# ericzzj1989/BALF

Measured on NVIDIA B200. Metric: images/sec detect+NMS+top-k @640x480, higher is better.
Workload: dtype fp16/tf32 operands (11-bit significand), fp32 accumulate

## Files before the change

### balf_b200/csrc/detector.cu

```cuda
#include <cuda_fp16.h>
#include "detector.cuh"

namespace balf {

constexpr int NT = 256;
constexpr int kWbufFloats = 4096;

enum { ACT_NONE = 0, ACT_RELU = 1, ACT_GELU = 2, ACT_LRELU = 3 };

template <int ACT> __device__ __forceinline__ float act_fn(float v) {
    if (ACT == ACT_RELU) return fmaxf(v, 0.0f);
    if (ACT == ACT_GELU) return 0.5f * v * (1.0f + erff(v * 0.70710678118654752440f));
    if (ACT == ACT_LRELU) return v > 0.0f ? v : 0.2f * v;
    return v;
}


template <int M, int K, int N, int ACT, bool ALIAS>
__device__ __forceinline__ void linear_tile(const float* in_s, const float* __restrict__ wT, int ldw,
                                            const float* __restrict__ bias, float* out_s, const float* res_s,
                                            float* wbuf) {
    constexpr int MP = M + 4;
    constexpr int TMB = M / 8, NTH = NT / TMB;
    constexpr int NC = N < NTH * 8 ? N : NTH * 8;
// ... 303 lines not shown
        float o = __ldg(w.ex2_b + c);
        for (int k = 0; k < C / 4; ++k) o = fmaf(hid[k], __ldg(w.ex2_w + (size_t)k * C + c), o);
        scale[(size_t)b * C + c] = 1.0f / (1.0f + expf(-o));
    }
}

template <int C, int swz, bool OH>
__global__ void pool_kernel(const float* __restrict__ r, const float* __restrict__ q, const float* __restrict__ scale,
                            int h, int w, float* __restrict__ out, size_t total) {
    size_t i = (size_t)blockIdx.x * blockDim.x + threadIdx.x;
    if (i >= total) return;
    constexpr int Q = C / 4;
    const int c4 = (int)(i % Q);
    size_t t = i / Q;
    const int wo = w / 2, ho = h / 2;
    const int px = (int)(t % wo);
    t /= wo;
    const int py = (int)(t % ho);
    const size_t b = t / ho;
    const float4 s = __ldg(reinterpret_cast<const float4*>(scale + b * C) + c4);
    float4 best = make_float4(kNegInf, kNegInf, kNegInf, kNegInf);
#pragma unroll
    for (int dy = 0; dy < 2; ++dy)
#pragma unroll
        for (int dx = 0; dx < 2; ++dx) {
            size_t p = (b * h + 2 * py + dy) * w + 2 * px + dx;
            const size_t rowi = p & 127;
            const size_t cs = (swz == 1 || swz == 2) ? (((p - rowi) * C) >> 2) + (size_t)(c4 >> 3) * (128 * 8) + rowi * 8 + ((c4 & 7) ^ (rowi & 7))
                                  : ((p * C) >> 2) + c4;
            float4 rv;
            if constexpr (swz == 1) {
                const uint2 h = __ldg(reinterpret_cast<const uint2*>(reinterpret_cast<const __half*>(r) + (p - rowi) * C +
                                                                     (size_t)(c4 >> 1) * (128 * 8) + rowi * 8 + (c4 & 1) * 4));
                const float2 lo = __half22float2(*reinterpret_cast<const __half2*>(&h.x)), hi = __half22float2(*reinterpret_cast<const __half2*>(&h.y));
                rv = make_float4(lo.x, lo.y, hi.x, hi.y);
            } else if constexpr (swz == 3) {
                const uint2 h = __ldg(reinterpret_cast<const uint2*>(reinterpret_cast<const __half*>(r) + p * C) + c4);
                const float2 lo = __half22float2(*reinterpret_cast<const __half2*>(&h.x)), hi = __half22float2(*reinterpret_cast<const __half2*>(&h.y));
                rv = make_float4(lo.x, lo.y, hi.x, hi.y);
            } else {
                rv = __ldg(reinterpret_cast<const float4*>(r) + cs);
            }
            float4 qv;
            if constexpr (swz == 1) {
                const unsigned char* qt = reinterpret_cast<const unsigned char*>(q) + (p - rowi) * C * 3;
                const uint2 t16 = __ldg(reinterpret_cast<const uint2*>(qt + ((size_t)(c4 >> 1) * 128 + rowi) * 16 + (c4 & 1) * 8));
                const uint32_t m8 = __ldg(reinterpret_cast<const uint32_t*>(qt + (size_t)128 * C * 2 + ((size_t)(c4 >> 2) * 128 + rowi) * 16 + (c4 & 3) * 4));
                qv.x = __uint_as_float(((t16.x & 0xFFFFu) << 16) | ((m8 & 0xFFu) << 8));
                qv.y = __uint_as_float((t16.x & 0xFFFF0000u) | (m8 & 0xFF00u));
                qv.z = __uint_as_float(((t16.y & 0xFFFFu) << 16) | ((m8 >> 8) & 0xFF00u));
                qv.w = __uint_as_float((t16.y & 0xFFFF0000u) | ((m8 >> 16) & 0xFF00u));
            } else {
                qv = __ldg(reinterpret_cast<const float4*>(q) + cs);
            }
            best.x = fmaxf(best.x, rv.x * s.x + qv.x); best.y = fmaxf(best.y, rv.y * s.y + qv.y);
            best.z = fmaxf(best.z, rv.z * s.z + qv.z); best.w = fmaxf(best.w, rv.w * s.w + qv.w);
        }
    if constexpr (OH) {
        uint2 o;
// ... 195 lines not shown
    {
        ProfScope p("det_se", st);
        se_kernel<C><<<Bc, kSeThreads, 0, st>>>(ws.partial, parts, 1.0f / (float)npix, w, ws.scale);
    }
    BALF_COUNT_LAUNCH(1);
    BALF_LAUNCH_OK();
    return 0;
}

template <int C>
static int run_pool(const Workspace& ws, int Bc, int h, int wd, float* out, cudaStream_t st, int swz = 0, bool oh = false) {
    size_t total = (size_t)Bc * (h / 2) * (wd / 2) * (C / 4);
    {
        ProfScope p("det_pool", st);
        const unsigned grid = (unsigned)((total + 255) / 256);
        if (swz == 1 && oh) pool_kernel<C, 1, true><<<grid, 256, 0, st>>>(ws.r, ws.q, ws.scale, h, wd, out, total);
        else if (swz == 1) pool_kernel<C, 1, false><<<grid, 256, 0, st>>>(ws.r, ws.q, ws.scale, h, wd, out, total);
        else if (swz == 2) pool_kernel<C, 2, false><<<grid, 256, 0, st>>>(ws.r, ws.q, ws.scale, h, wd, out, total);
        else if (swz == 3 && oh) pool_kernel<C, 3, true><<<grid, 256, 0, st>>>(ws.r, ws.q, ws.scale, h, wd, out, total);
        else if (swz == 3) pool_kernel<C, 3, false><<<grid, 256, 0, st>>>(ws.r, ws.q, ws.scale, h, wd, out, total);
        else if (oh) pool_kernel<C, 0, true><<<grid, 256, 0, st>>>(ws.r, ws.q, ws.scale, h, wd, out, total);
        else pool_kernel<C, 0, false><<<grid, 256, 0, st>>>(ws.r, ws.q, ws.scale, h, wd, out, total);
    }
    BALF_COUNT_LAUNCH(1);
    BALF_LAUNCH_OK();
    return 0;
}

}

using namespace balf;
// ... 96 lines not shown
    Workspace ws;
    ws_layout(a, chunk, Hp, Wp, workspace, &ws);
    const int nl = a.cell * a.cell + 1, hc = Hp / 8, wc = Wp / 8;
    if (int e = set_smem(head_kernel<256, 32>, HeadSmem<256, 32>::bytes)) return e;
    for (int b0 = 0; b0 < B; b0 += chunk) {
        const int Bc = B - b0 < chunk ? B - b0 : chunk;
        const float* xb = x + (size_t)b0 * 3 * Hp * Wp;
        const int tcm = precision >= 1 ? g_tc_mask : 0;
        const int px = precision == 2 ? 1 : 0;
        const DownW* d = w.down;
        int tiles = 0;
        if (tcm & 1) {
            if (int e = tc_run_level_dispatch(0, xb, true, d[0], a, tc_blob, Bc, Hp, Wp, ws.u, ws.v, ws.r, ws.q, ws.partial, st, px, 0)) return e;
            if (int e = run_se<32>(ws, d[0], Bc, Hp * Wp, Hp * Wp / 64, st)) return e;
        } else if (int e = run_level<3, 32, 128, 128>(xb, true, w.down[0], Bc, Hp, Wp, ws, st, &tiles)) return e;
        if (int e = run_pool<32>(ws, Bc, Hp, Wp, ws.pooled[0], st, (tcm & 1) ? 1 + px : 0, (tcm & 2) && !px)) return e;
        if (tcm & 2) {
            if (int e = tc_run_level_dispatch(1, ws.pooled[0], false, d[1], a, tc_blob, Bc, Hp / 2, Wp / 2, ws.u, ws.v, ws.r, ws.q, ws.partial, st, px, 0)) return e;
            if (int e = run_se<64>(ws, d[1], Bc, Hp * Wp / 4, Hp * Wp / 256, st)) return e;
        } else if (int e = run_level<32, 64, 128, 128>(ws.pooled[0], false, w.down[1], Bc, Hp / 2, Wp / 2, ws, st, &tiles)) return e;
        if (int e = run_pool<64>(ws, Bc, Hp / 2, Wp / 2, ws.pooled[1], st, (tcm & 2) ? 1 + px : 0, (tcm & 4) && !px)) return e;
        if (tcm & 4) {
            if (int e = tc_run_level_dispatch(2, ws.pooled[1], false, d[2], a, tc_blob, Bc, Hp / 4, Wp / 4, ws.u, ws.v, ws.r, ws.q, ws.partial, st, px, px == 0)) return e;
            if (int e = run_se<128>(ws, d[2], Bc, Hp * Wp / 16, Hp * Wp / 1024, st)) return e;
        } else if (int e = run_level<64, 128, 64, 64>(ws.pooled[1], false, w.down[2], Bc, Hp / 4, Wp / 4, ws, st, &tiles)) return e;
        if (int e = run_pool<128>(ws, Bc, Hp / 4, Wp / 4, ws.pooled[2], st, ((tcm & 4) && !px) ? 3 : 0, (tcm & 8) && !px)) return e;
        if (tcm & 8) {
            if (int e = tc_run_level_dispatch(3, ws.pooled[2], false, d[3], a, tc_blob, Bc, hc, wc, ws.u, ws.v, ws.r, ws.q, ws.partial, st, px, px == 0 && (tcm & 16) != 0)) return e;
            if (int e = run_se<256>(ws, d[3], Bc, hc * wc, hc * wc / 64, st)) return e;
        } else if (int e = run_level<128, 256, 64, 32>(ws.pooled[2], false, w.down[3], Bc, hc, wc, ws, st, &tiles)) return e;
        if (tcm & 16) {
// ... 17 lines not shown
```

### balf_b200/csrc/detector.cuh

```cuda
#pragma once
#include "common.cuh"
#include "../../include/balf_b200.h"

namespace balf {

constexpr int kHeadPad = 128;

struct DownW {
    const float *conv0_w, *conv0_b;
    const float *pn_w, *pn_b;
    const float *pd1_w, *pd1_b;
    struct Branch {
        const float *n_w, *n_b;
        const float *d1_w, *d1_b;
        const float *gn_w, *gn_b;
        const float *gd_w, *gd_b;
        const float *d2_w, *d2_b;
    } br[2];
    const float *pd2_w, *pd2_b;
    const float *rn_w, *rn_b;
    const float *rc1_w, *rc1_b, *rc2_w, *rc2_b;
    const float *ex0_w, *ex0_b;
    const float *ex2_w, *ex2_b;
    const float *c2_w, *c2_b;
// ... 37 lines not shown
        d.pd2_w = c.take(2 * ch * ch); d.pd2_b = c.take(ch);
        d.rn_w = c.take(ch); d.rn_b = c.take(ch);
        d.rc1_w = c.take(ch * ch); d.rc1_b = c.take(ch);
        d.rc2_w = c.take(ch * ch); d.rc2_b = c.take(ch);
        d.ex0_w = c.take(ch * red); d.ex0_b = c.take(red);
        d.ex2_w = c.take(red * ch); d.ex2_b = c.take(ch);
        d.c2_w = c.take(ch * ch); d.c2_b = c.take(ch);
    }
    const size_t cl = a.dims[4];
    w.head.w = c.take(cl * kHeadPad); w.head.b = c.take(kHeadPad);
    w.head.alpha = c.take(kHeadPad); w.head.beta = c.take(kHeadPad);
    if (out) *out = w;
    return c.off;
}

size_t tc_blob_floats(const balf_detector_arch& a);
int tc_pack_weights(const balf_detector_arch& a, const DetW& w, float* blob, cudaStream_t st);
int tc_run_level_dispatch(int level, const float* xin, bool nchw, const DownW& w, const balf_detector_arch& a, const float* blob,
                          int Bc, int h, int wd, float* u, float* v, float* r, float* q, float* partial, cudaStream_t st, int px, int r16);
int tc_run_head(const float* r, const float* q, const float* scale, const DownW& w, const HeadW& hw, const balf_detector_arch& a,
                const float* blob, int Bc, int hc, int wc, float* logits, float* prob, cudaStream_t st, int px, int r16);

}
```

### balf_b200/csrc/detector_tc.cuh

```cuda
#pragma once
#include <cuda_fp16.h>
#include "detector.cuh"
#include "umma.cuh"

namespace balf {
using namespace umma;

#ifndef BALF_EXP
#define BALF_EXP 0
#endif
#ifndef BALF_MERGE32_CTAS
#define BALF_MERGE32_CTAS 3
#endif
#ifndef BALF_MERGE_TPR
#define BALF_MERGE_TPR 2
#endif
#ifndef BALF_RC16_MINC
#define BALF_RC16_MINC 32
#endif
constexpr int TM = 128;
constexpr int NT2 = 256;
constexpr int kMaxSlot = 4;
constexpr int kMaxGemm = 6;

struct TcGemm {
    uint32_t goff;
    uint16_t nblk;
    uint16_t rows;
    uint16_t kb;
    uint16_t bias;
    uint16_t h16;
};
__host__ __device__ constexpr uint32_t tc_eb(int h16) { return h16 == 1 ? 2u : 4u; }
struct TcPlan {
    const float* base;
    TcGemm g[kMaxGemm];
    int ngemm;
    int resident;
// ... 108 lines not shown
};
template <int CIN, int C, int PX = 0> struct MergeG {
    static constexpr int count = MG_COUNT;
    static constexpr bool x3 = PX != 0;
    static constexpr bool ebias = C == 128 && PX == 0;
    static constexpr bool resident = PX ? C <= 32 : C <= 128;
    static constexpr int cap = 32768;
    static constexpr int nslot = PX ? (C == 64 ? 3 : 2) : (C == 256 ? 2 : 3);
    __host__ __device__ static constexpr int rows(int) { return C; }
    __host__ __device__ static constexpr int K(int gi) { return gi == MG_CONV0 ? tc_kin(CIN) : C; }
    __host__ __device__ static constexpr bool bias(int gi) { return !ebias && gi != MG_PD2A; }
    __host__ __device__ static constexpr bool h16(int gi) {
        return gi == MG_PD2A || gi == MG_PD2B || (gi == MG_CONV0 && CIN >= 8) || ((gi == MG_RC1 || gi == MG_RC2) && (PX || C > BALF_RC16_MINC));
    }
};
template <int C, int PX = 0> struct HeadG {
    static constexpr int count = HG_COUNT;
    static constexpr bool x3 = PX != 0;
    static constexpr bool resident = false;
    static constexpr int cap = 32768;
    static constexpr int nslot = 2;
    __host__ __device__ static constexpr int rows(int gi) { return gi == HG_DENSE ? kHeadN : C; }
    __host__ __device__ static constexpr int K(int) { return C; }
    __host__ __device__ static constexpr bool bias(int) { return true; }
    __host__ __device__ static constexpr bool h16(int) { return true; }
};
template <typename G> __host__ __device__ constexpr int g_mode(int gi) { return G::h16(gi) ? (G::x3 ? 2 : 1) : 0; }
template <typename G> __host__ __device__ constexpr uint32_t g_bytes(int gi) {
    return (uint32_t)G::rows(gi) * (G::K(gi) * tc_eb(g_mode<G>(gi)) + (G::bias(gi) ? 32u : 0u));
}
// ... 824 lines not shown
                const float mix_b1 = *mix_b1p;
                const unsigned long long b2 = pk2(mix_b1, mix_b1);
#pragma unroll
                for (int i = 0; i < SC; i += 2) upk2(mul2(pk2(y1[i], y1[i + 1]), add2(pk2(y2[i], y2[i + 1]), b2)), y2[i], y2[i + 1]);
                row_to_a16<SC, LOC>(y2, s.region, row, col0 + c);
            }
        }
        TC_TRACE(plan, it, 13);
        sync_for_mma<NG, NTG>(grp);
        if (!(BALF_EXP & 16) && w0 && elect_one()) { issue_linear_t<G, BG_D2>(ring, plan, region_addr, ones_addr, tm + Cfg::col_y, true); commit(s.done); }
        TC_TRACE(plan, it, 14);
        wait_done_ring<G, NG, NTG, Cfg::WW>(s.done, phase, ring, plan, w0, grp);
        TC_TRACE(plan, it, 15);
        {
            const bool odd = (threadIdx.x & 1) != 0;
            const size_t own_base = (Cfg::swz_out || Cfg::h16_out) ? ((size_t)img * npix + (pix & ~(TM - 1))) * C * (Cfg::h16_out && X3 ? 2 : 1)
                                                                   : ((size_t)img * npix + pix) * C;
            const int own_sw = pix & (TM - 1);
            const size_t oth_base = __shfl_xor_sync(0xffffffffu, (unsigned long long)own_base, 1);
            const int oth_sw = __shfl_xor_sync(0xffffffffu, own_sw, 1);
            const size_t base_a = odd ? oth_base : own_base, base_b = odd ? own_base : oth_base;
            const int sw_a = odd ? oth_sw : own_sw, sw_b = odd ? own_sw : oth_sw;
            if constexpr (CL16 && CH % 64 == 0) {
                float hv[CH / 2];
#pragma unroll
                for (int c = 0; c < CH; c += SC) {
                    float a[SC];
                    ld_row<SC>(lane_base + Cfg::col_y + col0 + c, a);
#pragma unroll
                    for (int j0 = 0; j0 < SC / 4; j0 += 8) {
                        float4 t8[8];
                        pair_load<8>(reinterpret_cast<const float4*>(orow + c) + j0, valid, t8);
#pragma unroll
// ... 366 lines not shown
    tc_finish(tm, Cfg::ncols);
}


template <int CIN, int C, int PX = 0> struct MergeBulkCfg {
    static constexpr int CH = C / 2;
    static constexpr bool cc0 = CIN < 8;
    static constexpr uint32_t tile_bytes = (uint32_t)TM * C * 4;
    static constexpr uint32_t uv_bytes = (uint32_t)TM * C * (PX ? 4u : 2u);
    static constexpr uint32_t r16_bytes = 0u;
    static constexpr uint32_t xbytes = cc0 ? 0u : (uint32_t)TM * tc_kin(CIN) * 4;
    static constexpr uint32_t region = 2 * uv_bytes + r16_bytes + 2 * tile_bytes + xbytes;
    static constexpr uint32_t xch = 2u * TM * 8u;
    static constexpr int col_acc = 0, col_x0 = C;
    static constexpr int ncols = tc_cols(cc0 ? C : 2 * C);
    static constexpr int min_ctas = C <= 32 ? (PX ? 2 : BALF_MERGE32_CTAS) : 1;
};

template <int CIN, int C, int PX = 0>
__global__ void __launch_bounds__(NT2, MergeBulkCfg<CIN, C, PX>::min_ctas)
tc_merge_bulk_kernel(const float* __restrict__ xin, DownW w, TcPlan plan, UnitGeom geo, const float* __restrict__ uin,
                     const float* __restrict__ vin, float* __restrict__ rout, float* __restrict__ qout, float* __restrict__ partial) {
    extern __shared__ __align__(1024) unsigned char smem[];
    using Cfg = MergeBulkCfg<CIN, C, PX>;
    constexpr int CH = Cfg::CH;
    using G = MergeG<CIN, C, PX>;
    constexpr int HM = PX ? 2 : 1, LOC = PX ? C / 8 : 0;
    constexpr bool XH = PX == 0 && CIN >= 8;
    constexpr int XM = XH ? 3 : HM;
    const TcShared s = carve(smem, Cfg::region, plan, 1, Cfg::xch);
    float* const regU = s.region;
// ... 165 lines not shown
            }
#pragma unroll
            for (int o = TPP / 2; o >= 1; o >>= 1) {
                acc.x += __shfl_xor_sync(0xffffffffu, acc.x, o);
                acc.y += __shfl_xor_sync(0xffffffffu, acc.y, o);
                acc.z += __shfl_xor_sync(0xffffffffu, acc.z, o);
                acc.w += __shfl_xor_sync(0xffffffffu, acc.w, o);
            }
            if (sub == 0) *reinterpret_cast<float4*>(partial + (size_t)(2 * t + uu) * C + ch * 4) = acc;
        }
    }
    if (w0 && elect_one()) bulk_wait_all();
    tc_finish(tm, Cfg::ncols);
}

template <int C, int PX = 0>
__global__ void __launch_bounds__(NT2, 1) tc_head_kernel(const float* __restrict__ r, const float* __restrict__ q,
                                                         const float* __restrict__ scale, TcPlan plan, UnitGeom geo, int cell,
                                                         float* __restrict__ logits, float* __restrict__ prob, int r16) {
    extern __shared__ __align__(1024) unsigned char smem[];
    using G = HeadG<C, PX>;
    constexpr int LOC = PX ? C / 8 : 0;
    constexpr uint32_t region_bytes = (uint32_t)TM * C * 4;
    constexpr int ncols = tc_cols(C + 96);
    constexpr int CH = C / 2;
    const TcShared s = carve(smem, region_bytes, plan);
    const int tid = threadIdx.x, row = tid & (TM - 1), half = tid >> 7;
    const int ntiles = (geo.total_units + 1) / 2;
    const uint32_t my_tiles = blockIdx.x < (unsigned)ntiles ? (ntiles - 1 - blockIdx.x) / gridDim.x + 1 : 0;
    Ring ring;
// ... 362 lines not shown
}


#ifdef BALF_TC_MAIN
int g_tc_variant = 0x41;
#else
extern int g_tc_variant;
#endif

template <int CIN, int C, int V, int PX>
static int tc_launch_branches(const float* xin, const DownW& w, const TcPlans& P, int level, const UnitGeom& g, int ntiles,
                              float* u, float* v, float* su, float* sv, cudaStream_t st) {
    using Cfg = typename BranchSel<C, V, PX>::Cfg;
    constexpr int NG = Cfg::groups;
    int grid = 0;
    for (int b = 0; b < 2; ++b) {
        const TcPlan& p = P.branch[level][b];
        const size_t smem = tc_smem_bytes(Cfg::region, p, NG, Cfg::xch);
        if (b == 0) {
            if (int e = tc_launch_cfg(tc_branch_kernel<CIN, C, 0, V, PX>, smem, tc_cols(Cfg::ncols * NG), ntiles, &grid, NG, Cfg::NTG)) return e;
            ProfScope ps(C == 32 ? "det_branch_grid_c32" : C == 64 ? "det_branch_grid_c64" : C == 128 ? "det_branch_grid_c128" : "det_branch_grid_c256", st);
            tc_branch_kernel<CIN, C, 0, V, PX><<<grid, Cfg::NTG * NG, smem, st>>>(xin, w, p, g, u, su);
        } else {
            if (int e = tc_launch_cfg(tc_branch_kernel<CIN, C, 1, V, PX>, smem, tc_cols(Cfg::ncols * NG), ntiles, &grid, NG, Cfg::NTG)) return e;
            ProfScope ps(C == 32 ? "det_branch_block_c32" : C == 64 ? "det_branch_block_c64" : C == 128 ? "det_branch_block_c128" : "det_branch_block_c256", st);
            tc_branch_kernel<CIN, C, 1, V, PX><<<grid, Cfg::NTG * NG, smem, st>>>(xin, w, p, g, v, sv);
        }
    }
    return 0;
}
template <int CIN, int C, int PX>
static int tc_run_branches(const float* xin, const DownW& w, const TcPlans& P, int level, const UnitGeom& g, int ntiles,
                           float* u, float* v, float* su, float* sv, cudaStream_t st) {
    const int var = (g_tc_variant >> (2 * level)) & 3;
    if constexpr (C == 32) {
        if (var == 1) return tc_launch_branches<CIN, C, 1, PX>(xin, w, P, level, g, ntiles, u, v, su, sv, st);
        if (var == 2) return tc_launch_branches<CIN, C, 2, PX>(xin, w, P, level, g, ntiles, u, v, su, sv, st);
    }
    if constexpr (C == 64 || C == 128 || C == 256) {
        if (var == 1) return tc_launch_branches<CIN, C, 1, PX>(xin, w, P, level, g, ntiles, u, v, su, sv, st);
    }
    return tc_launch_branches<CIN, C, 0, PX>(xin, w, P, level, g, ntiles, u, v, su, sv, st);
}

template <int CIN, int C, int PX>
static int tc_run_level(const float* xin, const DownW& w, const TcPlans& P, int level, int Bc, int h, int wd,
                        float* u, float* v, float* r, float* q, float* partial, cudaStream_t st, int r16) {
    (void)r16;
    UnitGeom g{h, wd, h / 8, wd / 8, h * wd / 64, Bc * (h * wd / 64), 1.0f / (float)(h * wd / 64), 1.0f / (float)(wd / 8), 1.0f / (float)(wd / 8)};
    BALF_REQUIRE(g.total_units < (1 << 23), "internal: %d units in one pass exceed the fast_div range", g.total_units);
    const int ntiles = (g.total_units + 1) / 2;
    int grid = 0;
    BALF_REQUIRE((plan_matches<BranchG<CIN, C, PX>>(P.branch[level][0]) && plan_matches<BranchG<CIN, C, PX>>(P.branch[level][1]) &&
                  plan_matches<MergeG<CIN, C, PX>>(P.merge[level])), "internal: compile-time and packed GEMM plans differ (level %d)", level);
    if (int e = tc_run_branches<CIN, C, PX>(xin, w, P, level, g, ntiles, u, v, r, q, st)) return e;
    if constexpr (C <= 64) {
        const TcPlan& p = P.merge[level];
        BALF_REQUIRE(g.total_units % 2 == 0, "internal: odd unit count at stage %d", level);
        const size_t smem = tc_smem_bytes(MergeBulkCfg<CIN, C, PX>::region, p, 1, MergeBulkCfg<CIN, C, PX>::xch);
        if (int e = tc_launch_cfg(tc_merge_bulk_kernel<CIN, C, PX>, smem, MergeBulkCfg<CIN, C, PX>::ncols, ntiles, &grid)) return e;
        ProfScope ps(C == 32 ? "det_merge_c32" : "det_merge_c64", st);
        tc_merge_bulk_kernel<CIN, C, PX><<<grid, NT2, smem, st>>>(xin, w, p, g, u, v, r, q, partial);
    } else {
        const TcPlan& p = P.merge[level];
        BALF_REQUIRE((!MergeCfg<C, PX>::bulk_uv || g.total_units % 2 == 0), "internal: odd unit count at stage %d", level);
        const size_t smem = tc_smem_bytes(MergeCfg<C, PX>::region, p, 1, MergeCfg<C, PX>::xch);
        if (int e = tc_launch_cfg(tc_merge_kernel<CIN, C, PX>, smem, MergeCfg<C, PX>::ncols, ntiles, &grid, 1, MergeCfg<C, PX>::NT)) return e;
        ProfScope ps(C == 128 ? "det_merge_c128" : "det_merge_c256", st);
        tc_merge_kernel<CIN, C, PX><<<grid, MergeCfg<C, PX>::NT, smem, st>>>(xin, w, p, g, u, v, r, q, partial, r16);
    }
    BALF_COUNT_LAUNCH(3);
    BALF_LAUNCH_OK();
    return 0;
}

template <int PX>
int tc_level_px(int level, const float* xin, const DownW& w, const balf_detector_arch& a, const float* blob,
                int Bc, int h, int wd, float* u, float* v, float* r, float* q, float* partial, cudaStream_t st, int r16) {
    TcPlans P;
    tc_build_plans(a, blob, &P, PX);
    switch (level) {
        case 0: return tc_run_level<3, 32, PX>(xin, w, P, 0, Bc, h, wd, u, v, r, q, partial, st, r16);
        case 1: return tc_run_level<32, 64, PX>(xin, w, P, 1, Bc, h, wd, u, v, r, q, partial, st, r16);
        case 2: return tc_run_level<64, 128, PX>(xin, w, P, 2, Bc, h, wd, u, v, r, q, partial, st, r16);
        default: return tc_run_level<128, 256, PX>(xin, w, P, 3, Bc, h, wd, u, v, r, q, partial, st, r16);
    }
// ... 52 lines not shown
```

Baseline: 5223.

## Fuse level-0 block branch with merge kernel and emit block-pixel layout for pool

For the first stage (C=32, default precision), the block-attention branch is now computed inside a new merge kernel. That kernel keeps the branch output in TMEM/shared memory instead of writing v to global memory and reading it back, which removes one launch and one global round-trip of the intermediate. The grid branch writes its output and the fused kernel writes r/q in a block-pixel tiled order, and the pool kernel gains a matching swz==4 index mode. The fused kernel processes chunks of 4 tiles to accumulate SE partial sums in shared memory. It uses more TMEM columns and shared memory per CTA, and requires the width to be a multiple of 64.

```diff
diff --git a/balf_b200/csrc/detector.cu b/balf_b200/csrc/detector.cu
--- a/balf_b200/csrc/detector.cu
+++ b/balf_b200/csrc/detector.cu
@@ -341,22 +341,36 @@
     const int c4 = (int)(i % Q);
     size_t t = i / Q;
     const int wo = w / 2, ho = h / 2;
-    const int px = (int)(t % wo);
-    t /= wo;
-    const int py = (int)(t % ho);
-    const size_t b = t / ho;
+    int px, py;
+    size_t b;
+    if constexpr (swz == 4) {
+        const int k = (int)(t & 31);
+        t >>= 5;
+        const int tw = w >> 4;
+        const size_t tpi = (size_t)(h >> 3) * tw;
+        b = t / tpi;
+        const int ti = (int)(t - b * tpi), by = ti / tw;
+        py = by * 4 + (k >> 3);
+        px = (ti - by * tw) * 8 + (k & 7);
+    } else {
+        px = (int)(t % wo);
+        t /= wo;
+        py = (int)(t % ho);
+        b = t / ho;
+    }
     const float4 s = __ldg(reinterpret_cast<const float4*>(scale + b * C) + c4);
     float4 best = make_float4(kNegInf, kNegInf, kNegInf, kNegInf);
+    const size_t p00 = swz == 4 ? b * h * w + bp_index(2 * py, 2 * px, w) : 0;
 #pragma unroll
     for (int dy = 0; dy < 2; ++dy)
 #pragma unroll
         for (int dx = 0; dx < 2; ++dx) {
-            size_t p = (b * h + 2 * py + dy) * w + 2 * px + dx;
+            const size_t p = swz == 4 ? p00 + 8 * dy + dx : (b * h + 2 * py + dy) * w + 2 * px + dx;
             const size_t rowi = p & 127;
-            const size_t cs = (swz == 1 || swz == 2) ? (((p - rowi) * C) >> 2) + (size_t)(c4 >> 3) * (128 * 8) + rowi * 8 + ((c4 & 7) ^ (rowi & 7))
+            const size_t cs = (swz == 1 || swz == 2 || swz == 4) ? (((p - rowi) * C) >> 2) + (size_t)(c4 >> 3) * (128 * 8) + rowi * 8 + ((c4 & 7) ^ (rowi & 7))
                                   : ((p * C) >> 2) + c4;
             float4 rv;
-            if constexpr (swz == 1) {
+            if constexpr (swz == 1 || swz == 4) {
                 const uint2 h = __ldg(reinterpret_cast<const uint2*>(reinterpret_cast<const __half*>(r) + (p - rowi) * C +
                                                                      (size_t)(c4 >> 1) * (128 * 8) + rowi * 8 + (c4 & 1) * 4));
                 const float2 lo = __half22float2(*reinterpret_cast<const __half2*>(&h.x)), hi = __half22float2(*reinterpret_cast<const __half2*>(&h.y));
@@ -369,7 +383,7 @@
                 rv = __ldg(reinterpret_cast<const float4*>(r) + cs);
             }
             float4 qv;
-            if constexpr (swz == 1) {
+            if constexpr (swz == 1 || swz == 4) {
                 const unsigned char* qt = reinterpret_cast<const unsigned char*>(q) + (p - rowi) * C * 3;
                 const uint2 t16 = __ldg(reinterpret_cast<const uint2*>(qt + ((size_t)(c4 >> 1) * 128 + rowi) * 16 + (c4 & 1) * 8));
                 const uint32_t m8 = __ldg(reinterpret_cast<const uint32_t*>(qt + (size_t)128 * C * 2 + ((size_t)(c4 >> 2) * 128 + rowi) * 16 + (c4 & 3) * 4));
@@ -595,7 +609,9 @@
     {
         ProfScope p("det_pool", st);
         const unsigned grid = (unsigned)((total + 255) / 256);
-        if (swz == 1 && oh) pool_kernel<C, 1, true><<<grid, 256, 0, st>>>(ws.r, ws.q, ws.scale, h, wd, out, total);
+        if (swz == 4 && oh) pool_kernel<C, 4, true><<<grid, 256, 0, st>>>(ws.r, ws.q, ws.scale, h, wd, out, total);
+        else if (swz == 4) pool_kernel<C, 4, false><<<grid, 256, 0, st>>>(ws.r, ws.q, ws.scale, h, wd, out, total);
+        else if (swz == 1 && oh) pool_kernel<C, 1, true><<<grid, 256, 0, st>>>(ws.r, ws.q, ws.scale, h, wd, out, total);
         else if (swz == 1) pool_kernel<C, 1, false><<<grid, 256, 0, st>>>(ws.r, ws.q, ws.scale, h, wd, out, total);
         else if (swz == 2) pool_kernel<C, 2, false><<<grid, 256, 0, st>>>(ws.r, ws.q, ws.scale, h, wd, out, total);
         else if (swz == 3 && oh) pool_kernel<C, 3, true><<<grid, 256, 0, st>>>(ws.r, ws.q, ws.scale, h, wd, out, total);
@@ -722,7 +738,7 @@
             if (int e = tc_run_level_dispatch(0, xb, true, d[0], a, tc_blob, Bc, Hp, Wp, ws.u, ws.v, ws.r, ws.q, ws.partial, st, px, 0)) return e;
             if (int e = run_se<32>(ws, d[0], Bc, Hp * Wp, Hp * Wp / 64, st)) return e;
         } else if (int e = run_level<3, 32, 128, 128>(xb, true, w.down[0], Bc, Hp, Wp, ws, st, &tiles)) return e;
-        if (int e = run_pool<32>(ws, Bc, Hp, Wp, ws.pooled[0], st, (tcm & 1) ? 1 + px : 0, (tcm & 2) && !px)) return e;
+        if (int e = run_pool<32>(ws, Bc, Hp, Wp, ws.pooled[0], st, (tcm & 1) ? (px ? 2 : 4) : 0, (tcm & 2) && !px)) return e;
         if (tcm & 2) {
             if (int e = tc_run_level_dispatch(1, ws.pooled[0], false, d[1], a, tc_blob, Bc, Hp / 2, Wp / 2, ws.u, ws.v, ws.r, ws.q, ws.partial, st, px, 0)) return e;
             if (int e = run_se<64>(ws, d[1], Bc, Hp * Wp / 4, Hp * Wp / 256, st)) return e;
diff --git a/balf_b200/csrc/detector.cuh b/balf_b200/csrc/detector.cuh
--- a/balf_b200/csrc/detector.cuh
+++ b/balf_b200/csrc/detector.cuh
@@ -75,6 +75,11 @@
     return c.off;
 }
 
+__host__ __device__ __forceinline__ int bp_index(int y, int x, int w) {
+    const int tok = (y & 7) * 8 + (x & 7);
+    return ((y >> 3) * (w >> 4) + (x >> 4)) * 128 + (tok >> 4) * 32 + ((x >> 3) & 1) * 16 + (tok & 15);
+}
+
 size_t tc_blob_floats(const balf_detector_arch& a);
 int tc_pack_weights(const balf_detector_arch& a, const DetW& w, float* blob, cudaStream_t st);
 int tc_run_level_dispatch(int level, const float* xin, bool nchw, const DownW& w, const balf_detector_arch& a, const float* blob,
diff --git a/balf_b200/csrc/detector_tc.cuh b/balf_b200/csrc/detector_tc.cuh
--- a/balf_b200/csrc/detector_tc.cuh
+++ b/balf_b200/csrc/detector_tc.cuh
@@ -8,9 +8,6 @@
 
 #ifndef BALF_EXP
 #define BALF_EXP 0
-#endif
-#ifndef BALF_MERGE32_CTAS
-#define BALF_MERGE32_CTAS 3
 #endif
 #ifndef BALF_MERGE_TPR
 #define BALF_MERGE_TPR 2
@@ -21,7 +18,7 @@
 constexpr int TM = 128;
 constexpr int NT2 = 256;
 constexpr int kMaxSlot = 4;
-constexpr int kMaxGemm = 6;
+constexpr int kMaxGemm = 11;
 
 struct TcGemm {
     uint32_t goff;
@@ -160,6 +157,20 @@
         return gi == MG_PD2A || gi == MG_PD2B || (gi == MG_CONV0 && CIN >= 8) || ((gi == MG_RC1 || gi == MG_RC2) && (PX || C > BALF_RC16_MINC));
     }
 };
+template <int C, int PX> constexpr bool kFusedBlockMerge = C == 32 && PX == 0;
+template <int CIN, int C> struct BlockMergeG {
+    using B = BranchG<CIN, C>;
+    using M = MergeG<CIN, C>;
+    static constexpr int count = BG_COUNT + MG_COUNT;
+    static constexpr bool x3 = false;
+    static constexpr bool resident = true;
+    static constexpr int cap = 32768;
+    static constexpr int nslot = 2;
+    __host__ __device__ static constexpr int rows(int gi) { return gi < BG_COUNT ? B::rows(gi) : M::rows(gi - BG_COUNT); }
+    __host__ __device__ static constexpr int K(int gi) { return gi < BG_COUNT ? B::K(gi) : M::K(gi - BG_COUNT); }
+    __host__ __device__ static constexpr bool bias(int gi) { return gi < BG_COUNT ? B::bias(gi) : M::bias(gi - BG_COUNT); }
+    __host__ __device__ static constexpr bool h16(int gi) { return gi < BG_COUNT ? B::h16(gi) : M::h16(gi - BG_COUNT); }
+};
 template <int C, int PX = 0> struct HeadG {
     static constexpr int count = HG_COUNT;
     static constexpr bool x3 = PX != 0;
@@ -1014,9 +1025,14 @@
         TC_TRACE(plan, it, 15);
         {
             const bool odd = (threadIdx.x & 1) != 0;
-            const size_t own_base = (Cfg::swz_out || Cfg::h16_out) ? ((size_t)img * npix + (pix & ~(TM - 1))) * C * (Cfg::h16_out && X3 ? 2 : 1)
+            int tpix = pix;
+            if constexpr (BR == 0 && kFusedBlockMerge<C, Cfg::PX>) {
+                const int un = valid ? 2 * t + ug - img * geo.upi : 0, fy = fast_div(un, geo.fw, geo.inv_fw), fx = un - fy * geo.fw;
+                tpix = bp_index((tok >> 3) * geo.fh + fy, (tok & 7) * geo.fw + fx, geo.w);
+            }
+            const size_t own_base = (Cfg::swz_out || Cfg::h16_out) ? ((size_t)img * npix + (tpix & ~(TM - 1))) * C * (Cfg::h16_out && X3 ? 2 : 1)
                                                                    : ((size_t)img * npix + pix) * C;
-            const int own_sw = pix & (TM - 1);
+            const int own_sw = tpix & (TM - 1);
             const size_t oth_base = __shfl_xor_sync(0xffffffffu, (unsigned long long)own_base, 1);
             const int oth_sw = __shfl_xor_sync(0xffffffffu, own_sw, 1);
             const size_t base_a = odd ? oth_base : own_base, base_b = odd ? own_base : oth_base;
@@ -1413,7 +1429,7 @@
     static constexpr uint32_t xch = 2u * TM * 8u;
     static constexpr int col_acc = 0, col_x0 = C;
     static constexpr int ncols = tc_cols(cc0 ? C : 2 * C);
-    static constexpr int min_ctas = C <= 32 ? (PX ? 2 : BALF_MERGE32_CTAS) : 1;
+    static constexpr int min_ctas = C <= 32 ? 2 : 1;
 };
 
 template <int CIN, int C, int PX = 0>
@@ -1609,6 +1625,302 @@
     tc_finish(tm, Cfg::ncols);
 }
 
+template <int C> struct BlockMergeCfg {
+    static constexpr int groups = 4;
+    static constexpr int NTG = TM;
+    static constexpr int chunk = 4;
+    static constexpr uint32_t a_bytes = (uint32_t)TM * C * 2;
+    static constexpr uint32_t w_bytes = (uint32_t)TM * C * 4;
+    static constexpr uint32_t q_bytes = (uint32_t)TM * C * 3;
+    static constexpr uint32_t s_bytes = 8u * 16u * C * 4u;
+    static constexpr uint32_t region = w_bytes + q_bytes + s_bytes;
+    static constexpr int col_u = 0, col_y = C, col_x0 = 3 * C;
+    static constexpr int ncols = 4 * C;
+};
+
+template <int CIN, int C>
+__global__ void __launch_bounds__(BlockMergeCfg<C>::NTG * BlockMergeCfg<C>::groups, 1)
+tc_block_merge_kernel(const float* __restrict__ xin, DownW w, TcPlan plan, UnitGeom geo, const float* __restrict__ uin,
+                      float* __restrict__ rout, float* __restrict__ qout, float* __restrict__ partial) {
+    extern __shared__ __align__(1024) unsigned char smem[];
+    using Cfg = BlockMergeCfg<C>;
+    using G = BlockMergeG<CIN, C>;
+    constexpr int NG = Cfg::groups, NTG = Cfg::NTG, CH = C;
+    constexpr int F_PD2A = BG_COUNT + MG_PD2A, F_PD2B = BG_COUNT + MG_PD2B, F_RC1 = BG_COUNT + MG_RC1, F_RC2 = BG_COUNT + MG_RC2;
+    static_assert(CIN < 8 && C == 32, "built for the network-input stage: conv.0 on the CUDA cores, one thread per 32-channel row");
+    static_assert(!G::h16(F_RC1) && !G::h16(F_RC2), "conv1 / conv2 read W as a tf32 swizzled-panel operand");
+    static_assert(2 * NG <= kMaxGroups, "completion and u' barriers per group");
+    static_assert(Cfg::ncols * NG <= 512, "TMEM columns");
+    TcShared s = carve(smem, Cfg::region, plan, NG, 0);
+    const int grp = (int)(threadIdx.x / NTG), row = (int)threadIdx.x - grp * NTG;
+    const int vblock = (int)blockIdx.x * NG + grp, vgrid = (int)gridDim.x * NG;
+    const int ntiles = geo.total_units / 2;
+    const int nchunks = ntiles / Cfg::chunk;
+    const uint32_t my_tiles = vblock < nchunks ? ((nchunks - 1 - vblock) / vgrid + 1) * Cfg::chunk : 0;
+    const DownW::Branch& br = w.br[1];
+    if (grp == 0) {
+        for (int i = row; i < C; i += NTG) { s.vec[i] = __ldg(br.gn_w + i); s.vec[256 + i] = __ldg(br.gn_b + i); }
+        for (int i = row; i < 64; i += NTG) s.vec[512 + i] = __ldg(br.gd_b + i) + 1.0f;
+        for (int i = row; i < CIN * C; i += NTG) s.vec[kConv0Off + i] = __ldg(w.conv0_w + i);
+        for (int i = row; i < C; i += NTG) s.vec[kConv0Off + CIN * C + i] = __ldg(w.conv0_b + i);
+    }
+    Ring ring;
+    const bool w0 = __shfl_sync(0xffffffffu, row >> 5, 0) == 0;
+    tc_prologue<G::nslot>(s, tc_cols(Cfg::ncols * NG), ring, plan, my_tiles, w0 && grp == 0);
+    if (grp > 0 && w0 && elect_one()) mbar_wait(&s.full[0], 0);
+    float* const regA = s.region + (size_t)grp * (Cfg::region / 4);
+    float* const regU = regA + Cfg::a_bytes / 4;
+    float* const regW = regA;
+    float* const regQ = regA + Cfg::w_bytes / 4;
+    float4* const regS = reinterpret_cast<float4*>(regQ + Cfg::q_bytes / 4);
+    uint64_t* const done = grp ? &s.gdone[grp] : s.done;
+    uint64_t* const ld_u = &s.gdone[NG + grp];
+    const uint32_t tm = *s.tmem_slot + (uint32_t)(grp * Cfg::ncols);
+    const uint32_t lane_base = tm + ((uint32_t)(row & ~31) << 16);
+    const uint32_t a_addr = smem_u32(regA), u_addr = smem_u32(regU), q_addr = smem_u32(regQ), ones_addr = smem_u32(s.ones);
+    const int ug = (row & 31) >> 4, tok = (row >> 5) * 16 + (row & 15);
+    const float* const mix_b1p = s.vec + 512 + tok;
+    const size_t npix = (size_t)geo.h * geo.w;
+    const size_t tile_floats = (size_t)TM * C;
+    uint32_t phase = 0, ld_phase = 0;
+    InputPf<CIN, 1> pf;
+    auto coords = [&](int tt, int& im, int& px) {
+        const int un = 2 * tt + ug;
+        im = fast_div(un, geo.upi, geo.inv_upi);
+        px = unit_pixel<1>(geo, un - im * geo.upi, tok);
+    };
+    auto load_u = [&](int tt) {
+        mbar_expect_tx(ld_u, Cfg::a_bytes);
+        bulk_load(u_addr, uin + (size_t)tt * (Cfg::a_bytes / 4), Cfg::a_bytes, ld_u);
+    };
+    auto stats_of = [&](const float (&v)[CH], int c0, int n, float& sum, float& sq) {
+        unsigned long long s2 = pk2(0.f, 0.f), q2 = pk2(0.f, 0.f);
+#pragma unroll
+        for (int i = 0; i < n; i += 2) {
+            const unsigned long long x = pk2(v[c0 + i], v[c0 + i + 1]);
+            s2 = add2(s2, x); q2 = fma2(x, x, q2);
+        }
+        float a, b;
+        upk2(s2, a, b); sum = a + b;
+        upk2(q2, a, b); sq = a + b;
+    };
+    float4* const my_s = regS + (size_t)(tok >> 3) * (C / 4) * 16 + ug * 8 + (tok & 7);
+    const int t_first = vblock * Cfg::chunk;
+    if (t_first < ntiles) {
+        int im, px;
+        coords(t_first, im, px);
+        fetch_input_row<CIN, true, 1>(xin, npix, (size_t)im, px, true, 0, pf);
+        if (w0 && elect_one()) load_u(t_first);
+    }
+    for (int t = t_first, nt; t < ntiles; t = nt) {
+        const int kc = t % Cfg::chunk;
+        nt = kc + 1 < Cfg::chunk ? t + 1 : t + 1 + (vgrid - 1) * Cfg::chunk;
+        float v[CH], rstd, shift;
+        {
+            const float4 xv = pf.v[0];
+            if (nt < ntiles) {
+                int im, px;
+                coords(nt, im, px);
+                fetch_input_row<CIN, true, 1>(xin, npix, (size_t)im, px, true, 0, pf);
+            }
+            conv0_row<CIN, C, CH>(xv, s.vec, 0, v);
+            st_row<CH>(lane_base + Cfg::col_x0, v);
+            float sum, sq;
+            stats_of(v, 0, CH, sum, sq);
+            row_stats<NG, 1>(sum, sq, nullptr, row, 0, C, rstd, shift, grp);
+            norm_row<CH>(v, rstd, shift);
+            row_to_a16<CH>(v, regA, row, 0);
+        }
+        sync_for_mma<NG, NTG>(grp);
+        if (w0 && elect_one()) { issue_linear_t<G, BG_PD1>(ring, plan, a_addr, ones_addr, tm + Cfg::col_u, true); commit(done); }
+        wait_done_ring<G, NG, NTG>(done, phase, ring, plan, w0, grp);
+        {
+            ld_row<CH>(lane_base + Cfg::col_u, v);
+            float sum = 0.f, sq = 0.f;
+            gelu_row<CH, true>(v, sum, sq);
+            st_row<CH>(lane_base + Cfg::col_u, v);
+            row_stats<NG, 1>(sum, sq, nullptr, row, 0, C, rstd, shift, grp);
+            norm_row<CH>(v, rstd, shift);
+            row_to_a16<CH>(v, regA, row, 0);
+        }
+        sync_for_mma<NG, NTG>(grp);
+        if (w0 && elect_one()) {
+            issue_linear_t<G, BG_D1A>(ring, plan, a_addr, ones_addr, tm + Cfg::col_y, true);
+            issue_linear_t<G, BG_D1B>(ring, plan, a_addr, ones_addr, tm + Cfg::col_y + C, true);
+            commit(done);
+        }
+        wait_done_ring<G, NG, NTG>(done, phase, ring, plan, w0, grp);
+        {
+            ld_row<CH>(lane_base + Cfg::col_y, v);
+            { float d0, d1; gelu_row<CH, false>(v, d0, d1); }
+            st_row<CH>(lane_base + Cfg::col_y, v);
+            ld_row<CH>(lane_base + Cfg::col_y + C, v);
+            float sum = 0.f, sq = 0.f;
+            gelu_row<CH, true>(v, sum, sq);
+            row_stats<NG, 1>(sum, sq, nullptr, row, 0, C, rstd, shift, grp);
+            norm_row<CH>(v, rstd, shift);
+#pragma unroll
+            for (int i = 0; i < CH; i += 4) {
+                const float4 gw = *reinterpret_cast<const float4*>(s.vec + i), gb = *reinterpret_cast<const float4*>(s.vec + 256 + i);
+                upk2(fma2(pk2(v[i], v[i + 1]), pk2(gw.x, gw.y), pk2(gb.x, gb.y)), v[i], v[i + 1]);
+                upk2(fma2(pk2(v[i + 2], v[i + 3]), pk2(gw.z, gw.w), pk2(gb.z, gb.w)), v[i + 2], v[i + 3]);
+            }
+            row_to_a16<CH>(v, regA, row, 0);
+        }
+        sync_for_mma<NG, NTG>(grp);
+        if (w0 && elect_one()) { issue_mix_t<G, BG_WM, C>(ring, plan, a_addr, tm + Cfg::col_y + C); commit(done); }
+        wait_done_ring<G, NG, NTG>(done, phase, ring, plan, w0, grp);
+        {
+            constexpr int SC = 16;
+#pragma unroll 1
+            for (int c = 0; c < CH; c += SC) {
+                float y1[SC], y2[SC];
+                ld_row<SC>(lane_base + Cfg::col_y + c, y1);
+                ld_row<SC>(lane_base + Cfg::col_y + C + c, y2);
+                const float mix_b1 = *mix_b1p;
+                const unsigned long long b2 = pk2(mix_b1, mix_b1);
+#pragma unroll
+                for (int i = 0; i < SC; i += 2) upk2(mul2(pk2(y1[i], y1[i + 1]), add2(pk2(y2[i], y2[i + 1]), b2)), y2[i], y2[i + 1]);
+                row_to_a16<SC>(y2, regA, row, c);
+            }
+        }
+        sync_for_mma<NG, NTG>(grp);
+        if (w0 && elect_one()) { issue_linear_t<G, BG_D2>(ring, plan, a_addr, ones_addr, tm + Cfg::col_y, true); commit(done); }
+        wait_done_ring<G, NG, NTG>(done, phase, ring, plan, w0, grp);
+        {
+            float r[CH];
+            ld_row<CH>(lane_base + Cfg::col_y, v);
+            ld_row<CH>(lane_base + Cfg::col_u, r);
+#pragma unroll
+            for (int i = 0; i < CH; i += 2) upk2(add2(pk2(v[i], v[i + 1]), pk2(r[i], r[i + 1])), v[i], v[i + 1]);
+            row_to_a16<CH>(v, regA, row, 0);
+        }
+        sync_for_mma<NG, NTG>(grp);
+        if (w0 && elect_one()) {
+            mbar_wait(ld_u, ld_phase & 1);
+            fence_after_sync();
+            issue_linear_t<G, F_PD2A>(ring, plan, u_addr, ones_addr, tm + Cfg::col_y, true);
+            issue_linear_t<G, F_PD2B>(ring, plan, a_addr, ones_addr, tm + Cfg::col_y, false);
+            commit(done);
+            bulk_wait_read();
+        }
+        ++ld_phase;
+        wait_done_ring<G, NG, NTG>(done, phase, ring, plan, w0, grp);
+        {
+            float x0[CH];
+            ld_row<CH>(lane_base + Cfg::col_y, v);
+            ld_row<CH>(lane_base + Cfg::col_x0, x0);
+#pragma unroll
+            for (int i = 0; i < CH; i += 2) {
+                const unsigned long long xz = pk2(x0[i], x0[i + 1]);
+                const unsigned long long x1 = add2(pk2(v[i], v[i + 1]), xz);
+                upk2(x1, v[i], v[i + 1]);
+                upk2(add2(x1, xz), x0[i], x0[i + 1]);
+            }
+            unsigned char* const qb = reinterpret_cast<unsigned char*>(regQ);
+#pragma unroll
+            for (int j = 0; j < CH / 8; ++j) {
+                uint32_t bq[8];
+#pragma unroll
+                for (int e = 0; e < 8; ++e) bq[e] = __float_as_uint(x0[8 * j + e]) + 0x80u;
+                uint4 o;
+                o.x = __byte_perm(bq[0], bq[1], 0x7632); o.y = __byte_perm(bq[2], bq[3], 0x7632);
+                o.z = __byte_perm(bq[4], bq[5], 0x7632); o.w = __byte_perm(bq[6], bq[7], 0x7632);
+                *reinterpret_cast<uint4*>(qb + ((size_t)j * TM + row) * 16) = o;
+            }
+#pragma unroll
+            for (int j = 0; j < CH / 16; ++j) {
+                uint32_t w4[4];
+#pragma unroll
+                for (int e = 0; e < 4; ++e) {
+                    const uint32_t b0 = __float_as_uint(x0[16 * j + 4 * e]) + 0x80u, b1 = __float_as_uint(x0[16 * j + 4 * e + 1]) + 0x80u;
+                    const uint32_t b2 = __float_as_uint(x0[16 * j + 4 * e + 2]) + 0x80u, b3 = __float_as_uint(x0[16 * j + 4 * e + 3]) + 0x80u;
+                    w4[e] = __byte_perm(__byte_perm(b0, b1, 0x0051), __byte_perm(b2, b3, 0x0051), 0x5410);
+                }
+                *reinterpret_cast<uint4*>(qb + (size_t)TM * C * 2 + ((size_t)j * TM + row) * 16) = make_uint4(w4[0], w4[1], w4[2], w4[3]);
+            }
+            float sum0, sq0, sum1, sq1;
+            stats_of(v, 0, CH / 2, sum0, sq0);
+            stats_of(v, CH / 2, CH / 2, sum1, sq1);
+            row_stats<NG, 1>(sum0 + sum1, sq0 + sq1, nullptr, row, 0, C, rstd, shift, grp);
+            norm_row<CH>(v, rstd, shift);
+            row_to_sw<CH, true>(v, regW, row, 0);
+        }
+        sync_for_mma<NG, NTG>(grp);
+        if (w0 && elect_one()) {
+            issue_linear_t<G, F_RC1, true>(ring, plan, smem_u32(regW), ones_addr, tm + Cfg::col_y, true);
+            commit(done);
+            bulk_store(qout + (size_t)t * (tile_floats * 3 / 4), q_addr, Cfg::w_bytes / 4 * 3);
+            bulk_commit();
+        }
+        wait_done_ring<G, NG, NTG>(done, phase, ring, plan, w0, grp);
+        ld_row<CH>(lane_base + Cfg::col_y, v);
+#pragma unroll
+        for (int i = 0; i < CH; i += 2) {
+            float l0, l1;
+            upk2(mul2(pk2(v[i], v[i + 1]), pk2(0.2f, 0.2f)), l0, l1);
+            v[i] = fmaxf(v[i], l0); v[i + 1] = fmaxf(v[i + 1], l1);
+        }
+        row_to_sw<CH, true>(v, regW, row, 0);
+        sync_for_mma<NG, NTG>(grp);
+        if (w0 && elect_one()) {
+            issue_linear_t<G, F_RC2, true>(ring, plan, smem_u32(regW), ones_addr, tm + Cfg::col_y, true);
+            commit(done);
+            bulk_wait_read();
+        }
+        wait_done_ring<G, NG, NTG>(done, phase, ring, plan, w0, grp);
+        if (nt < ntiles && w0 && elect_one()) load_u(nt);
+        ld_row<CH>(lane_base + Cfg::col_y, v);
+#pragma unroll
+        for (int j = 0; j < CH / 4; ++j) {
+            float4 a = make_float4(v[4 * j], v[4 * j + 1], v[4 * j + 2], v[4 * j + 3]);
+            if (kc > 0) {
+                const float4 o = my_s[j * 16];
+                a = make_float4(o.x + a.x, o.y + a.y, o.z + a.z, o.w + a.w);
+            }
+            my_s[j * 16] = a;
+        }
+        {
+            __half* rt = reinterpret_cast<__half*>(regQ) + (size_t)row * 8;
+#pragma unroll
+            for (int j = 0; j < CH / 8; ++j) {
+                uint32_t h[4];
+#pragma unroll
+                for (int e = 0; e < 4; ++e)
+                    asm("cvt.rn.satfinite.f16x2.f32 %0, %1, %2;" : "=r"(h[e]) : "f"(v[8 * j + 2 * e + 1]), "f"(v[8 * j + 2 * e]));
+                *reinterpret_cast<uint4*>(rt + (size_t)j * (TM * 8)) = make_uint4(h[0], h[1], h[2], h[3]);
+            }
+        }
+        sync_for_mma<NG, NTG>(grp);
+        if (w0 && elect_one()) {
+            bulk_store(rout + (size_t)t * (tile_floats / 2), q_addr, Cfg::a_bytes);
+            bulk_commit();
+        }
+        if (kc + 1 == Cfg::chunk) {
+            constexpr int CQ = C / 4;
+            const int t0 = t - kc, im = fast_div(2 * t0, geo.upi, geo.inv_upi);
+            const int u0 = 2 * t0 - im * geo.upi, by = fast_div(u0, geo.w >> 3, geo.inv_bw), bx = u0 - by * (geo.w >> 3);
+            const size_t unit0 = (size_t)im * geo.upi + (size_t)by * 8 * (geo.w >> 6) + (bx >> 3);
+            const int sub = row & 15;
+#pragma unroll 1
+            for (int pr = row >> 4; pr < 8 * CQ; pr += NTG / 16) {
+                const int yy = pr / CQ, ch = pr % CQ;
+                float4 acc = regS[(size_t)pr * 16 + sub];
+#pragma unroll
+                for (int o = 8; o >= 1; o >>= 1) {
+                    acc.x += __shfl_xor_sync(0xffffffffu, acc.x, o);
+                    acc.y += __shfl_xor_sync(0xffffffffu, acc.y, o);
+                    acc.z += __shfl_xor_sync(0xffffffffu, acc.z, o);
+                    acc.w += __shfl_xor_sync(0xffffffffu, acc.w, o);
+                }
+                if (sub == 0) *reinterpret_cast<float4*>(partial + (unit0 + (size_t)yy * (geo.w >> 6)) * C + ch * 4) = acc;
+            }
+        }
+    }
+    if (w0 && elect_one()) bulk_wait_all();
+    tc_finish(*s.tmem_slot, tc_cols(Cfg::ncols * NG));
+}
+
 template <int C, int PX = 0>
 __global__ void __launch_bounds__(NT2, 1) tc_head_kernel(const float* __restrict__ r, const float* __restrict__ q,
                                                          const float* __restrict__ scale, TcPlan plan, UnitGeom geo, int cell,
@@ -2001,14 +2313,14 @@
     using Cfg = typename BranchSel<C, V, PX>::Cfg;
     constexpr int NG = Cfg::groups;
     int grid = 0;
-    for (int b = 0; b < 2; ++b) {
+    for (int b = 0; b < (kFusedBlockMerge<C, PX> ? 1 : 2); ++b) {
         const TcPlan& p = P.branch[level][b];
         const size_t smem = tc_smem_bytes(Cfg::region, p, NG, Cfg::xch);
         if (b == 0) {
             if (int e = tc_launch_cfg(tc_branch_kernel<CIN, C, 0, V, PX>, smem, tc_cols(Cfg::ncols * NG), ntiles, &grid, NG, Cfg::NTG)) return e;
             ProfScope ps(C == 32 ? "det_branch_grid_c32" : C == 64 ? "det_branch_grid_c64" : C == 128 ? "det_branch_grid_c128" : "det_branch_grid_c256", st);
             tc_branch_kernel<CIN, C, 0, V, PX><<<grid, Cfg::NTG * NG, smem, st>>>(xin, w, p, g, u, su);
-        } else {
+        } else if constexpr (!kFusedBlockMerge<C, PX>) {
             if (int e = tc_launch_cfg(tc_branch_kernel<CIN, C, 1, V, PX>, smem, tc_cols(Cfg::ncols * NG), ntiles, &grid, NG, Cfg::NTG)) return e;
             ProfScope ps(C == 32 ? "det_branch_block_c32" : C == 64 ? "det_branch_block_c64" : C == 128 ? "det_branch_block_c128" : "det_branch_block_c256", st);
             tc_branch_kernel<CIN, C, 1, V, PX><<<grid, Cfg::NTG * NG, smem, st>>>(xin, w, p, g, v, sv);
@@ -2028,6 +2340,18 @@
         if (var == 1) return tc_launch_branches<CIN, C, 1, PX>(xin, w, P, level, g, ntiles, u, v, su, sv, st);
     }
     return tc_launch_branches<CIN, C, 0, PX>(xin, w, P, level, g, ntiles, u, v, su, sv, st);
+}
+
+static TcPlan tc_block_merge_plan(const TcPlan& b, const TcPlan& m) {
+    TcPlan p = b;
+    for (int i = 0; i < m.ngemm; ++i) p.g[b.ngemm + i] = m.g[i];
+    p.ngemm = b.ngemm + m.ngemm;
+    p.resident = 1;
+    p.bytes = b.bytes + m.bytes;
+    p.slot_bytes = b.slot_bytes > m.slot_bytes ? b.slot_bytes : m.slot_bytes;
+    p.nslot = 2;
+    p.trace = nullptr;
+    return p;
 }
 
 template <int CIN, int C, int PX>
@@ -2040,23 +2364,37 @@
     int grid = 0;
     BALF_REQUIRE((plan_matches<BranchG<CIN, C, PX>>(P.branch[level][0]) && plan_matches<BranchG<CIN, C, PX>>(P.branch[level][1]) &&
                   plan_matches<MergeG<CIN, C, PX>>(P.merge[level])), "internal: compile-time and packed GEMM plans differ (level %d)", level);
-    if (int e = tc_run_branches<CIN, C, PX>(xin, w, P, level, g, ntiles, u, v, r, q, st)) return e;
-    if constexpr (C <= 64) {
-        const TcPlan& p = P.merge[level];
-        BALF_REQUIRE(g.total_units % 2 == 0, "internal: odd unit count at stage %d", level);
-        const size_t smem = tc_smem_bytes(MergeBulkCfg<CIN, C, PX>::region, p, 1, MergeBulkCfg<CIN, C, PX>::xch);
-        if (int e = tc_launch_cfg(tc_merge_bulk_kernel<CIN, C, PX>, smem, MergeBulkCfg<CIN, C, PX>::ncols, ntiles, &grid)) return e;
-        ProfScope ps(C == 32 ? "det_merge_c32" : "det_merge_c64", st);
-        tc_merge_bulk_kernel<CIN, C, PX><<<grid, NT2, smem, st>>>(xin, w, p, g, u, v, r, q, partial);
+    if constexpr (kFusedBlockMerge<C, PX>) {
+        using Cfg = BlockMergeCfg<C>;
+        const TcPlan p = tc_block_merge_plan(P.branch[level][1], P.merge[level]);
+        BALF_REQUIRE(wd % 64 == 0, "internal: level width %d is not a multiple of 64 (chunks of block-pair tiles)", wd);
+        BALF_REQUIRE((plan_matches<BlockMergeG<CIN, C>>(p)), "internal: compile-time and packed GEMM plans differ (level %d, block + merge)", level);
+        if (int e = tc_run_branches<CIN, C, PX>(xin, w, P, level, g, ntiles, u, nullptr, r, nullptr, st)) return e;
+        const size_t smem = tc_smem_bytes(Cfg::region, p, Cfg::groups, 0);
+        if (int e = tc_launch_cfg(tc_block_merge_kernel<CIN, C>, smem, tc_cols(Cfg::ncols * Cfg::groups), ntiles / Cfg::chunk, &grid, Cfg::groups, Cfg::NTG)) return e;
+        {
+            ProfScope ps(C == 32 ? "det_block_merge_c32" : "det_block_merge_c64", st);
+            tc_block_merge_kernel<CIN, C><<<grid, Cfg::NTG * Cfg::groups, smem, st>>>(xin, w, p, g, u, r, q, partial);
+        }
     } else {
-        const TcPlan& p = P.merge[level];
-        BALF_REQUIRE((!MergeCfg<C, PX>::bulk_uv || g.total_units % 2 == 0), "internal: odd unit count at stage %d", level);
-        const size_t smem = tc_smem_bytes(MergeCfg<C, PX>::region, p, 1, MergeCfg<C, PX>::xch);
-        if (int e = tc_launch_cfg(tc_merge_kernel<CIN, C, PX>, smem, MergeCfg<C, PX>::ncols, ntiles, &grid, 1, MergeCfg<C, PX>::NT)) return e;
-        ProfScope ps(C == 128 ? "det_merge_c128" : "det_merge_c256", st);
-        tc_merge_kernel<CIN, C, PX><<<grid, MergeCfg<C, PX>::NT, smem, st>>>(xin, w, p, g, u, v, r, q, partial, r16);
-    }
-    BALF_COUNT_LAUNCH(3);
+        if (int e = tc_run_branches<CIN, C, PX>(xin, w, P, level, g, ntiles, u, v, r, q, st)) return e;
+        if constexpr (C <= 64) {
+            const TcPlan& p = P.merge[level];
+            BALF_REQUIRE(g.total_units % 2 == 0, "internal: odd unit count at stage %d", level);
+            const size_t smem = tc_smem_bytes(MergeBulkCfg<CIN, C, PX>::region, p, 1, MergeBulkCfg<CIN, C, PX>::xch);
+            if (int e = tc_launch_cfg(tc_merge_bulk_kernel<CIN, C, PX>, smem, MergeBulkCfg<CIN, C, PX>::ncols, ntiles, &grid)) return e;
+            ProfScope ps(C == 32 ? "det_merge_c32" : "det_merge_c64", st);
+            tc_merge_bulk_kernel<CIN, C, PX><<<grid, NT2, smem, st>>>(xin, w, p, g, u, v, r, q, partial);
+        } else {
+            const TcPlan& p = P.merge[level];
+            BALF_REQUIRE((!MergeCfg<C, PX>::bulk_uv || g.total_units % 2 == 0), "internal: odd unit count at stage %d", level);
+            const size_t smem = tc_smem_bytes(MergeCfg<C, PX>::region, p, 1, MergeCfg<C, PX>::xch);
+            if (int e = tc_launch_cfg(tc_merge_kernel<CIN, C, PX>, smem, MergeCfg<C, PX>::ncols, ntiles, &grid, 1, MergeCfg<C, PX>::NT)) return e;
+            ProfScope ps(C == 128 ? "det_merge_c128" : "det_merge_c256", st);
+            tc_merge_kernel<CIN, C, PX><<<grid, MergeCfg<C, PX>::NT, smem, st>>>(xin, w, p, g, u, v, r, q, partial, r16);
+        }
+    }
+    BALF_COUNT_LAUNCH((kFusedBlockMerge<C, PX> ? 2 : 3));
     BALF_LAUNCH_OK();
     return 0;
 }
```

New measurement: 5330, median of 6. 2.0% higher.
